# moble/scri

Hardware: AMD Instinct MI355X
Metric: timesteps/sec for full BMS transform, l_max=16, 1e5 steps; fp64 (higher is better)
Workload: dtype f64

## Files before the change

### scri_amd/csrc/engine.h

```cpp
#pragma once
#include <algorithm>
#include <array>
#include <cmath>
#include <chrono>
#include <cstdarg>
#include <cstdio>
#include <cstdlib>
#include <cstring>
#include <functional>
#include <map>
#include <new>
#include <string>
#include <thread>
#include <vector>

#include "../../include/scri_amd.h"
#include "kernels.h"
#include "pixel_math.h"
#include "wigner.h"

using namespace bms;

#define BMS_INTERNAL __attribute__((visibility("hidden")))

// ... 87 lines not shown
  int64_t n = 0, lo = 0, hi = 0, j0 = 0, j1 = 0;
  std::vector<double> host;
  const double* pending = nullptr;
  bool walked = false, regular = true;
  double* d_x = nullptr;
  BsplineTable* d_tab = nullptr;
  BsplineForward* d_fwd = nullptr;
};
struct PixelCache {
  bool valid = false, in_use = false, hit = false;
  uint64_t gen = 0;
  std::string key;
  PixelTables T;
  DevPixel D;
  bool B_valid = false;
  int B_spin = 0, B_ell_min = 0, B_ell_max = 0, B_cols = 0;
  double* d_B = nullptr;
  bool B5_valid = false, B5_sigma = false;
  int B5_ell_max = 0, B5_cols = 0;
  double* d_B5[5] = {nullptr, nullptr, nullptr, nullptr, nullptr};
  bool win_valid = false, win_abd = false;
  uint64_t win_tgen = 0, win_pgen = 0;
  int64_t win_lo = 0, win_hi = 0;
};

struct bms_ctx {
  int device = 0;
  hipStream_t own_stream = nullptr;
  hipStream_t stream = nullptr;
  hipStream_t aux = nullptr;
  std::string err;
  RouteOptions opt;
  uint64_t ws_limit = 96ull << 30;
  bool ws_limit_set = false;
  uint64_t sticky_limit = 0;
  int sticky_left = 0;
  unsigned long long* d_eval_stats = nullptr;
  uint64_t eval_tiles = 0;
  bool alloc_failed = false;
  std::map<std::string, DevBuf> bufs;
  std::vector<Slab> slabs;
  int delta_lmax = -1;
  int delta_mfma_lmax = -1;
  uint64_t rot_launches[3] = {0, 0, 0};
  int rot_valu_waves = 0;
  hipStream_t pipe_up = nullptr, pipe_down = nullptr;
// ... 5 lines not shown
  size_t pix_back_cap = 0;
  hipEvent_t ev_tables = nullptr, ev_aux_done = nullptr;
  double* rot_ring_dev = nullptr;
  int rot_ring_next = 0;
  std::map<std::pair<int, int>, RotResPlan> rot_res_plans;
  int n_cu = 0;
  std::map<std::string, std::pair<std::array<int, 6>, AnalysisPlan>> plans;
  std::map<std::array<int, 5>, SynthesisPlan> syn_plans;
  double ring_key[9] = {0, 0, 0, 0, 0, 0, 0, 0, 0};
  int ring_verdict = -1;
  std::vector<double> ring_thetas;
  std::map<std::array<int, 5>, std::pair<std::vector<double>, SynthesisPlan>> syn_plans_axis;
  bool timing = false;
  struct Timed {
    int tag;
    hipEvent_t a, b;
  };
  std::vector<Timed> timed;
  std::vector<hipEvent_t> event_pool;
  double tag_ms[BMS_TAG_COUNT] = {0};
  long long tag_calls[BMS_TAG_COUNT] = {0};
  TimeAxisCache tcache;
  PixelCache pcache;
};

static inline void note_alloc_failure(bms_ctx* c) {
  if (c) c->alloc_failed = true;
}

struct ScopedTimer {
  bms_ctx* c;
  int tag;
  hipStream_t stream;
  hipEvent_t a = nullptr, b = nullptr;
  static hipEvent_t get(bms_ctx* c) {
    if (!c->event_pool.empty()) {
      hipEvent_t e = c->event_pool.back();
      c->event_pool.pop_back();
      return e;
    }
    hipEvent_t e = nullptr;
    (void)hipEventCreate(&e);
    return e;
  }
  ScopedTimer(bms_ctx* c_, int tag_, hipStream_t stream_ = nullptr) : c(c_), tag(tag_), stream(stream_ ? stream_ : c_->stream) {
    if (c->timing) {
// ... 283 lines not shown
  c->tcache.in_use = c->tcache.hit = false;
  c->tcache.pending = nullptr;
  c->pcache.in_use = c->pcache.hit = false;
}
inline int reuse_tag(const bms_shard* sh) { return 1 + ((sh && sh->col_parts > 1 && sh->col_part >= 0) ? 1 + (sh->col_part & 0x7fff) + ((sh->col_parts & 0x7fff) << 15) : 0); }
struct KnotTables {
  double* d_x = nullptr;
  SplineTable* d_tab = nullptr;
  BsplineTable* d_bstab = nullptr;
  BsplineForward* d_bsfwd = nullptr;
  bool times_ahead = false;
  bool axis_known = false;
};
struct ChunkPlan {
  int64_t chunk = 0;
  int spline_tile = SPLINE_TILE;
};
BMS_INTERNAL int knot_tables_ahead(bms_ctx* c, const double* t, int64_t n, const bms_shard* sh, int64_t t_lo, int64_t t_hi, KnotTables& kt);
BMS_INTERNAL int knot_tables_of_call(bms_ctx* c, const double* t, int64_t n, int64_t t_lo, int64_t t_hi, int64_t row0, int64_t rows_avail, bool bsg, PieceTables* shared, KnotTables& kt);
BMS_INTERNAL int refuse_sharded_graded_axis(bms_ctx* c, bool regular_mesh, const bms_shard* sh, int64_t n);
BMS_INTERNAL int plan_chunks(bms_ctx* c, uint64_t ws_limit, double bytes_per_row, int64_t n_new, bool regular_mesh, int64_t n, const char* how_many, int n_cols, ChunkPlan& P);
BMS_INTERNAL int chunk_rows(bms_ctx* c, const PixelTables& T, const double* t, int64_t n, bool regular_mesh, int64_t c0, int64_t c1, int64_t row0, int64_t rows_avail, int64_t& g0, int64_t& g1);
BMS_INTERNAL int rotate_into_grid_frame(bms_ctx* c, const bms_transformation* tr, double* data, int64_t rows, int64_t ld, int ell_min, int ell_max);
BMS_INTERNAL int rotated_input_in_grid_frame(bms_ctx* c, const bms_transformation* tr, const char* name, int mem, const double** d_data, int64_t rows, int64_t ld, int ell_min, int ell_max);
BMS_INTERNAL int spline_eval_args(bms_ctx* c, const KnotTables& kt, const PixelTables& T, int cA, int cB, const double* t, int64_t n, int64_t g0, int64_t g1, int64_t c0, int64_t c1,
                                  double* out, long long ldo, long long ldg, SplineEval& ev);
BMS_INTERNAL void time_axis_commit(bms_ctx* c, bool walked, bool regular);
BMS_INTERNAL void drop_setup_caches(bms_ctx* c);
BMS_INTERNAL bool cached_window(bms_ctx* c, bool abd, int64_t& i_lo, int64_t& i_hi);
BMS_INTERNAL void keep_window(bms_ctx* c, bool abd, int64_t i_lo, int64_t i_hi);
BMS_INTERNAL int stage_in(bms_ctx* c, const char* name, const void* src, int mem, size_t bytes, const double** dev);
BMS_INTERNAL void time_window(int64_t n, const bms_shard* sh, int64_t& lo, int64_t& hi);
BMS_INTERNAL int validate_transformation(bms_ctx* c, int64_t n, const double* t, const bms_transformation* tr, int64_t n_min);
BMS_INTERNAL int walk_time_axis(bms_ctx* c, const double* t, int64_t lo, int64_t hi, bool* regular);
BMS_INTERNAL int validate_common(bms_ctx* c, int64_t n, const double* t, const bms_transformation* tr, int64_t lo = 0, int64_t hi = -1,
                           bool* regular = nullptr, int64_t n_min = 4);
BMS_INTERNAL int spline_tile_for(const double* x, int64_t n);
BMS_INTERNAL BsplineSpread skew_spread(const PixelTables& T, int cA, int cB, const double* x_host);
BMS_INTERNAL int eval_search_halfwidth(const PixelTables& T, int cA, int cB, const double* x_host, int64_t g0, int64_t g1);
BMS_INTERNAL bool large_synthesis_route(const bms_ctx* c, int n_theta, int n_phi, int ell_min, int ell_max);
BMS_INTERNAL bool axis_boost_pays(const bms_ctx* c, int n_modes, int n_theta, int n_phi);
BMS_INTERNAL bool separable_rotor_grid(const bms_transformation* tr, std::vector<double>& thetas, bool axis_boost_off = false);
BMS_INTERNAL bool separable_rotor_grid(bms_ctx* c, const bms_transformation* tr, std::vector<double>& thetas);
BMS_INTERNAL int build_synthesis(bms_ctx* c, int n_theta, int n_phi, int spin, int ell_min, int ell_max, SynthesisPlan& P,
                           const std::vector<double>* thetas = nullptr);
BMS_INTERNAL int run_synthesis(bms_ctx* c, const SynthesisPlan& P, const double* A, long long lda, long long rows, const double* off, double* Y,
                         long long ldy, const double* scale = nullptr);
BMS_INTERNAL int column_plan(const bms_ctx* c, const bms_transformation* tr, int n_out);
BMS_INTERNAL int device_pixel_tables(bms_ctx* c, const bms_transformation* tr, PixelTables& T, int mode, int spin, int cw,
                               const std::vector<cplx>* coef0, const std::vector<cplx>* coef1, const cplx cv[4], DevPixel& D,
                               int plan, hipStream_t PS = nullptr,
                               const std::function<int(hipStream_t, const DevPixel&, int)>& behind_tables = nullptr,
                               const std::function<void()>& while_waiting = nullptr, int reuse = 0);
BMS_INTERNAL int tables_and_window(bms_ctx* c, const bms_transformation* tr, const double* t, int64_t n, bool abd, PixelTables& T, int64_t& i_lo,
                                   int64_t& i_hi);
BMS_INTERNAL int column_range(bms_ctx* c, const bms_shard* sh, int n_cols, int& cA, int& cB);
BMS_INTERNAL int part_analysis_matrix(bms_ctx* c, const AnalysisPlan& A, const char* name, int n_cols, const int* col_of_pixel,
                                double** d_At, long long* ld_at);
BMS_INTERNAL uint64_t eval_tile_count(long long rows, int n_cols, int step);
BMS_INTERNAL int rotate_impl(bms_ctx* c, void* data, int mem, int64_t n_times, int64_t ld, int ell_min, int ell_max, const void* spinors, bool series,
                             bool sync_after = true);
```

### scri_amd/csrc/engine_modes.hip

```cpp
#include "engine.h"

constexpr int SYN_EVAL_MIN_ELL = 15;

struct PointwiseWM {
  const double* d_off = nullptr;
  const double* d_scale = nullptr;
  int n_aux = 0;
  double coeff[4];
  int power[4];
  const double *d_alpha = nullptr, *d_xa = nullptr, *d_xb = nullptr;
};

extern "C" int bms_transform_modes(bms_ctx* c, const bms_wm_input* in, const bms_transformation* tr, double* t_out,
                                   void* data_out, int64_t* n_times_out) try {
  return bms_transform_modes_shard(c, in, tr, nullptr, t_out, data_out, n_times_out, nullptr);
} BMS_CATCH(c)

extern "C" int bms_shard_plan(bms_ctx* c, const double* t, int64_t n, const bms_transformation* tr, int64_t out_i0,
                              int64_t out_i1, int64_t need_rows[2], int64_t window[2]) try {
  if (!t || !tr || !need_rows || !window) return fail(c, BMS_ERR_INVALID, "NULL argument");
  int rc = validate_common(c, n, t, tr);
  if (rc) return rc;
  PixelTables T;
  build_pixel_tables(tr, T);
// ... 349 lines not shown
    const bool want_syn_eval = c->opt.on(OPT_SYNTHESIS_EVAL) || (!c->opt.on(OPT_NO_SYNTHESIS_EVAL) && in->ell_max >= SYN_EVAL_MIN_ELL);
    if (sep && no_boost && bs && syn.nt != 0 && rows_avail >= 8 && in->t && want_syn_eval &&
        synthesis_eval_supported(syn.g, syn.nt, &se_lds, &se_nph, &se_rr, &se_xw)) {
      double bound = 0.0;
      for (int l = 1; l <= lst; ++l)
        for (int m = -l; m <= l; ++m) {
          const cplx a = st[LM_index(l, m, 0)];
          bound += std::sqrt(a.re * a.re + a.im * a.im) * std::sqrt((2 * l + 1) / (4 * M_PI));
        }
      const int64_t r0 = row0, r1 = row0 + rows_avail;
      double dx = (in->t[r1 - 1] - in->t[r0]) / (double)(r1 - 1 - r0);
      for (int64_t k = r0; k + 64 < r1; k += 64) dx = std::min(dx, (in->t[k + 64] - in->t[k]) / 64.0);
      syn_eval = dx > 0.0 && 2.0 * bound / dx <= (se_xw >= 1024 ? 384.0 : 160.0);
      for (int l = 0; l <= lst && !coef0.empty(); ++l)
        for (int m = -l; m <= l; ++m) {
          const cplx a = coef0[LM_index(l, m, 0)];
          if ((a.re != 0 || a.im != 0) && (l < in->ell_min || l > in->ell_max)) syn_eval = false;
        }
    }
  }
  std::vector<int> term_col;
  std::vector<double> term_val;
  double* d_Ac = nullptr;
  if (gemm_eval || syn_eval) {
    if ((rc = dev_buf_t(c, "Afull", (size_t)rows_avail * ld_af, &d_Ac))) return rc;
    if (c->opt.on(OPT_TWO_SWEEPS)) {
      if ((rc = dev_buf_t(c, "Afwd", (size_t)rows_avail * ld_af, &d_Af))) return rc;
      TIMED(c, BMS_TAG_SPLINE_FORWARD, launch_bspline_forward_modes(S, F[0].d_data, F[0].ld * 2, n_modes, d_Af, ld_af, row0, rows_avail, n, kt.d_bsfwd,
                                                                    SPLINE_TILE, SPLINE_HALO, 1));
      TIMED(c, BMS_TAG_SPLINE_BACKWARD, launch_bspline_backward_modes(S, d_Af, ld_af, n_modes + 1, d_Ac, ld_af, row0, rows_avail, kt.d_bstab, SPLINE_TILE, SPLINE_HALO));
    } else
      TIMED(c, BMS_TAG_SPLINE_FORWARD, launch_bspline_solve_modes(S, F[0].d_data, F[0].ld * 2, n_modes, d_Ac, ld_af, row0, rows_avail, kt.d_bsfwd, kt.d_bstab, 1));
    if (syn_eval && !coef0.empty()) {
      for (int l = in->ell_min; l <= std::min(lst, in->ell_max); ++l)
        for (int m = -l; m <= l; ++m) {
          const cplx a = coef0[LM_index(l, m, 0)];
          if (a.re == 0 && a.im == 0) continue;
          term_col.push_back(LM_index(l, m, in->ell_min));
          term_val.push_back(a.re);
          term_val.push_back(a.im);
        }
      if (!term_col.empty()) {
        void *vc, *vv;
        if ((rc = upload(c, "term_col", term_col.data(), sizeof(int) * term_col.size(), &vc))) return rc;
        if ((rc = upload(c, "term_val", term_val.data(), sizeof(double) * term_val.size(), &vv))) return rc;
        TIMED(c, BMS_TAG_POINTWISE, launch_sub_const_modes(S, d_Ac, ld_af, rows_avail, (int)term_col.size(), (const int*)vc, (const double*)vv, n_modes));
      }
    }
  } else if (bs && rows_avail > 0) {
    if ((rc = dev_buf_t(c, "Afwd", (size_t)rows_avail * ld_af, &d_Af))) return rc;
    TIMED(c, BMS_TAG_SPLINE_FORWARD, launch_bspline_forward_modes(S, F[0].d_data, F[0].ld * 2, n_modes, d_Af, ld_af, row0, rows_avail, n, kt.d_bsfwd,
                                                                  SPLINE_TILE, SPLINE_HALO, 1));
  }
  trace.mark("elimination / solve on the modes (enqueue)");
  if (sep && (rc = rotate_into_grid_frame(c, tr, syn_eval ? d_Ac : d_Af, rows_avail, ld_af / 2, in->ell_min, in->ell_max))) return rc;
  SynthesisPlan syn_f[5];
  bool sep_fields = false;
  if (!bs && rows_avail >= 1 && !(sh && sh->col_parts > 1) && tr->n_theta >= 3 && !c->opt.on(OPT_NO_SEPARABLE_SYNTHESIS) &&
      (no_boost || (axis_boost_pays(c, n_modes, tr->n_theta, tr->n_phi) && separable_rotor_grid(c, tr, ring_theta)))) {
    sep_fields = true;
    for (int fi = 0; fi < 1 + (psi ? in->n_aux : 0) && sep_fields; ++fi) {
      const int f_spin = fi ? in->aux_spin[fi - 1] : s, f_lo = fi ? in->aux_ell_min[fi - 1] : in->ell_min, f_hi = fi ? in->aux_ell_max[fi - 1] : in->ell_max;
      if (f_lo < 0 || f_hi < f_lo) {
        sep_fields = false;
        break;
      }
      if ((rc = build_synthesis(c, tr->n_theta, tr->n_phi, f_spin, f_lo, f_hi, syn_f[fi], no_boost ? nullptr : &ring_theta))) return rc;
      sep_fields = syn_f[fi].large;
    }
  }
  PixelTables T;
  DevPixel DP;
  const int col_plan = (grid_out || sep || sep_fields) ? 0 : column_plan(c, tr, n_out);
  bool B_built = false;
  if (shared && c->piece_tables_valid) {
    if (shared->col_plan != col_plan)
      return fail(c, BMS_ERR_UNSUPPORTED, "a piece of the pipelined call chose another synthesis route than the first one (column plan %d vs %d)",
                  col_plan, shared->col_plan);
// ... 252 lines not shown
```

### scri_amd/csrc/engine_rotate.hip

```cpp
#include "engine.h"


constexpr int ROT_RING = 64;

static hipError_t copy_block(char* host, int64_t ld, double* dev, int64_t n_modes, int64_t n_times, int blocks, int k, bool up, hipStream_t s) {
  const int64_t r0 = n_times * k / blocks, rows = n_times * (k + 1) / blocks - r0;
  const size_t row_bytes = (size_t)n_modes * 16, pitch = (size_t)ld * 16;
  char* h = host + (size_t)r0 * pitch;
  return up ? hipMemcpy2DAsync(dev, row_bytes, h, pitch, row_bytes, (size_t)rows, hipMemcpyHostToDevice, s)
            : hipMemcpy2DAsync(h, pitch, dev, row_bytes, row_bytes, (size_t)rows, hipMemcpyDeviceToHost, s);
}
int rotate_impl(bms_ctx* c, void* data, int mem, int64_t n_times, int64_t ld, int ell_min, int ell_max, const void* spinors, bool series,
                bool sync_after) {
  if (!c) return BMS_ERR_INVALID;
  if (!valid_mem(mem)) return fail(c, BMS_ERR_INVALID, "mem is BMS_HOST or BMS_DEVICE, got %d", mem);
  HIP_TRY(c, hipSetDevice(c->device));
  if (n_times < 0 || ell_min < 0 || ell_max < ell_min) return fail(c, BMS_ERR_INVALID, "bad sizes");
  if (ell_max > MAX_ELL) return fail(c, BMS_ERR_UNSUPPORTED, "ell_max = %d is beyond %d", ell_max, MAX_ELL);
  const int64_t n_modes = LM_total_size(ell_min, ell_max);
  if (ld < n_modes) return fail(c, BMS_ERR_INVALID, "row stride %lld smaller than %lld modes", (long long)ld, (long long)n_modes);
  if (n_times == 0) return BMS_OK;
  if (!data) return fail(c, BMS_ERR_INVALID, "NULL data");
  struct Segment {
    int lo, hi, kind;
    RotResPlan plan;
    size_t lds;
    const double* tab;
  };
  std::vector<Segment> segs;
  int rc = BMS_OK;
  {
    const bool allow_res = !c->opt.on(OPT_ROTATE_VALU) && !c->opt.on(OPT_ROTATE_STAGED) && ld * 256 <= 0x7ffe0000LL;
    int l = ell_min;
    while (l <= ell_max) {
      Segment sg{};
      bool placed = false;
// ... 12 lines not shown
        }
      }
      if (!placed) {
        sg.lo = l;
        sg.hi = ell_max;
        sg.kind = (rotate_mfma_supported(ell_max) && !c->opt.on(OPT_ROTATE_VALU)) ? 1 : 2;
        if (sg.kind == 2 && rotate_waves_per_block(ell_max) < 1)
          return fail(c, BMS_ERR_UNSUPPORTED, "ell_max=%d too large for the rotation kernels", ell_max);
      }
      segs.push_back(sg);
      l = sg.hi + 1;
    }
  }
  const double* d_delta = nullptr;
  const long long* d_off = nullptr;
  if (segs.back().kind != 0) {
    rc = segs.back().kind == 1 ? ensure_delta_mfma(c, ell_max, &d_delta, &d_off) : ensure_delta(c, ell_max, &d_delta, &d_off);
    if (rc) return rc;
  }
  double* d_data = (double*)data;
  const double* d_rot = (const double*)spinors;
  const size_t data_bytes = ((size_t)(n_times - 1) * ld + n_modes) * 16;
  const size_t rot_bytes = (series ? (size_t)n_times : 1) * 32;
  auto launch_segments = [&](double* base, int64_t rows, int64_t pitch, const double* rot) -> int {
    for (const Segment& sg : segs) {
      double* seg_data = base + 2 * ((long long)sg.lo * sg.lo - (long long)ell_min * ell_min);
      if (sg.kind == 0)
        TIMED(c, BMS_TAG_ROTATE, launch_rotate_modes_resident(c->stream, seg_data, rows, pitch, rot, series ? 4 : 0, sg.tab, sg.plan, sg.lds, nullptr, c->n_cu));
      else if (sg.kind == 1)
        TIMED(c, BMS_TAG_ROTATE, launch_rotate_modes_mfma(c->stream, seg_data, rows, pitch, sg.lo, sg.hi, rot, series ? 4 : 0, d_delta, d_off));
      else
        TIMED(c, BMS_TAG_ROTATE, launch_rotate_modes(c->stream, seg_data, rows, pitch, sg.lo, sg.hi, rot, series ? 4 : 0, d_delta, d_off, &c->rot_valu_waves));
      if (rows > 0) ++c->rot_launches[sg.kind];
    }
    return BMS_OK;
  };
  const size_t row_bytes = (size_t)n_modes * 16;
  int blocks = c->opt.on(OPT_NO_ROTATE_PIPELINE) ? 1 : (int)std::min<size_t>(16, (size_t)n_times * row_bytes / (12u << 20));
  if (const char* e = BMS_PROBE_ENV("SCRI_AMD_ROTATE_BLOCKS")) blocks = atoi(e);
  if (mem == BMS_HOST && blocks >= 2 && n_times >= 64 * blocks) {
    const int64_t rows_max = (n_times + blocks - 1) / blocks;
    double* d_buf[2];
    if ((rc = dev_buf_t(c, "rot_pipe0", (size_t)rows_max * n_modes * 2, &d_buf[0]))) return rc;
    if ((rc = dev_buf_t(c, "rot_pipe1", (size_t)rows_max * n_modes * 2, &d_buf[1]))) return rc;
    const double* d_r = nullptr;
    {
      double* r = nullptr;
      if ((rc = dev_buf_t(c, "rot_spinors", rot_bytes / 8, &r))) return rc;
      HIP_TRY(c, hipMemcpyAsync(r, spinors, rot_bytes, hipMemcpyHostToDevice, c->stream));
      d_r = r;
    }
    const char* err = "rotation of a host series in blocks";
    return run_host_pipeline(
        c, 0, blocks, true, false, err, err,
        [&](int k, int slot) { return copy_block((char*)data, ld, d_buf[slot], n_modes, n_times, blocks, k, true, c->pipe_up); },
        [&](int k, int slot) {
// ... 157 lines not shown
```

### scri_amd/csrc/engine_tables.hip

```cpp
#include "engine.h"


void build_rotor_grid(const double fr[4], const double v[3], int n_theta, int n_phi, std::vector<Quat>& R) {
  R.resize((size_t)n_theta * n_phi);
  const Quat frq = {fr[0], fr[1], fr[2], fr[3]};
  const BoostSpec bs = make_boost_spec(v);
  for (int j = 0; j < n_theta; ++j)
    for (int k = 0; k < n_phi; ++k) R[(size_t)j * n_phi + k] = pixel_rotor(frq, bs, j, k, n_theta, n_phi);
}

void theta_quadrature_weights(int n_theta, std::vector<double>& q) {
  const int M = 2 * n_theta - 2;
  q.assign(n_theta, 0.0);
  for (int j = 0; j < n_theta; ++j) {
    const double th = M_PI * j / (n_theta - 1);
    double E = 0.0;
    for (int p = -M / 2 + 1; p <= M / 2; ++p)
      if ((p & 1) == 0) E += 2.0 / (1.0 - (double)p * p) * std::cos(p * th);
    q[j] = (2 * M_PI / M) * E * ((j == 0 || j == n_theta - 1) ? 1.0 : 2.0);
  }
}

template <class T>
void delta_matrix(int ell, std::vector<double>& D ) {
// ... 453 lines not shown
    K.walked = false, K.regular = true;
    K.pending = t + lo;
    K.in_use = true;
  }
  return BMS_OK;
}

void time_axis_commit(bms_ctx* c, bool walked, bool regular) {
  TimeAxisCache& K = c->tcache;
  if (!K.in_use) return;
  if (K.pending) {
    K.host.assign(K.pending, K.pending + (K.hi - K.lo));
    K.pending = nullptr;
    K.valid = true;
  }
  if (walked && K.valid) K.walked = true, K.regular = regular;
}

void drop_setup_caches(bms_ctx* c) {
  c->tcache.valid = c->tcache.in_use = c->tcache.hit = false;
  c->tcache.pending = nullptr;
  c->pcache.valid = c->pcache.in_use = c->pcache.hit = false;
  c->pcache.B_valid = c->pcache.B5_valid = c->pcache.win_valid = false;
}

static bool window_keepable(const bms_ctx* c) {
  const TimeAxisCache& A = c->tcache;
  return A.in_use && c->pcache.in_use && A.lo == 0 && A.hi == A.n;
}
bool cached_window(bms_ctx* c, bool abd, int64_t& i_lo, int64_t& i_hi) {
  const PixelCache& P = c->pcache;
  if (!window_keepable(c) || !c->tcache.hit || !P.hit || !P.win_valid || P.win_abd != abd || P.win_tgen != c->tcache.gen || P.win_pgen != P.gen)
    return false;
  i_lo = P.win_lo, i_hi = P.win_hi;
  return true;
}
void keep_window(bms_ctx* c, bool abd, int64_t i_lo, int64_t i_hi) {
  PixelCache& P = c->pcache;
  if (!window_keepable(c)) return;
  P.win_valid = true, P.win_abd = abd, P.win_tgen = c->tcache.gen, P.win_pgen = P.gen, P.win_lo = i_lo, P.win_hi = i_hi;
}

int stage_in(bms_ctx* c, const char* name, const void* src, int mem, size_t bytes, const double** dev) {
  if (mem == BMS_DEVICE) {
    *dev = (const double*)src;
    return BMS_OK;
// ... 480 lines not shown
  return BMS_OK;
}

int chunk_rows(bms_ctx* c, const PixelTables& T, const double* t, int64_t n, bool regular_mesh, int64_t c0, int64_t c1, int64_t row0,
               int64_t rows_avail, int64_t& g0, int64_t& g1) {
  g0 = 0, g1 = n;
  if (regular_mesh) needed_rows(T, t, n, c0, c1, g0, g1);
  if (g0 < row0 || g1 > row0 + rows_avail)
    return fail(c, BMS_ERR_INVALID,
                "shard holds rows [%lld, %lld) but outputs [%lld, %lld) need rows [%lld, %lld): halo too small "
                "(use bms_shard_plan)",
                (long long)row0, (long long)(row0 + rows_avail), (long long)c0, (long long)c1, (long long)g0, (long long)g1);
  return BMS_OK;
}

static bool identity_rotor(const double* q) { return q[0] == 1.0 && q[1] == 0.0 && q[2] == 0.0 && q[3] == 0.0; }
int rotate_into_grid_frame(bms_ctx* c, const bms_transformation* tr, double* data, int64_t rows, int64_t ld, int ell_min, int ell_max) {
  const double* q = tr->frame_rotation;
  if (identity_rotor(q)) return BMS_OK;
  const double sp[4] = {q[0], q[3], q[2], q[1]};
  return rotate_impl(c, data, BMS_DEVICE, rows, ld, ell_min, ell_max, sp, false, false);
}

int rotated_input_in_grid_frame(bms_ctx* c, const bms_transformation* tr, const char* name, int mem, const double** d_data, int64_t rows, int64_t ld,
                                int ell_min, int ell_max) {
  double* d_copy = const_cast<double*>(*d_data);
  if (mem == BMS_DEVICE && !identity_rotor(tr->frame_rotation)) {
    int rc;
    if ((rc = dev_buf_t(c, name, (size_t)rows * ld * 2, &d_copy))) return rc;
    HIP_TRY(c, hipMemcpyAsync(d_copy, *d_data, (size_t)rows * ld * 16, hipMemcpyDeviceToDevice, c->stream));
    *d_data = d_copy;
  }
  return rotate_into_grid_frame(c, tr, d_copy, rows, ld, ell_min, ell_max);
}

int spline_eval_args(bms_ctx* c, const KnotTables& kt, const PixelTables& T, int cA, int cB, const double* t, int64_t n, int64_t g0, int64_t g1,
                     int64_t c0, int64_t c1, double* out, long long ldo, long long ldg, SplineEval& ev) {
  ev.table = kt.d_bstab, ev.x = kt.d_x, ev.tt = T.tt, ev.g0 = g0, ev.n_knots = n;
  ev.i_lo = c0, ev.i_hi = c1, ev.out = out, ev.ldo = ldo;
  ev.search_halfwidth = eval_search_halfwidth(T, cA, cB, t, g0, g1);
  ev.inv_dx = (g1 - g0 >= 2 && t[g1 - 1] > t[g0]) ? (double)(g1 - 1 - g0) / (t[g1 - 1] - t[g0]) : 0.0;
  ev.side = nullptr, ev.side_ld = ldg;
  if (!c->d_eval_stats) {
    HIP_TRY(c, hipMalloc(&c->d_eval_stats, 16));
    HIP_TRY(c, hipMemsetAsync(c->d_eval_stats, 0, 16, c->stream));
  }
// ... 7 lines not shown
```

### scri_amd/csrc/kernels.h

```cpp
#pragma once
#include <algorithm>
#include <vector>
#include <hip/hip_runtime.h>
#include <stdint.h>

#include "env.h"

#include <map>
#include <mutex>
#include <utility>

namespace bms {

constexpr long long GRID_Y_MAX = 65535;

inline int lds_per_workgroup(int dev) {
  int lds = 0, v = 0;
  if (hipDeviceGetAttribute(&v, hipDeviceAttributeSharedMemPerBlockOptin, dev) == hipSuccess) lds = std::max(lds, v);
  if (hipDeviceGetAttribute(&v, hipDeviceAttributeMaxSharedMemoryPerBlock, dev) == hipSuccess) lds = std::max(lds, v);
  (void)hipGetLastError();
  if (lds <= 64 * 1024) lds = 160 * 1024;
  return lds;
}

// ... 162 lines not shown
                                       long long g0, long long n_rows, long long n_knots, const double* x,
                                       const SplineTable* table, int tile, int halo, const double* base,
                                       const double* skew_a, const double* skew_b, double tt, long long i_lo,
                                       long long i_hi, double* out, long long ldo);

struct BsplineTable {
  double m[16];
  double G, D;
  double x;
  double pad;
};
struct BsplineForward {
  double P, A, E, x;
};
hipError_t launch_bspline_table(hipStream_t stream, const double* x, long long n, BsplineTable* table, BsplineForward* fwd,
                                long long j_lo , long long j0, long long j1);
hipError_t launch_bspline_forward_modes(hipStream_t stream, const double* A, long long lda, int n_modes, double* Aout,
                                        long long ldo, long long g0, long long n_rows, long long n_knots,
                                        const BsplineForward* table, int tile, int halo, int with_ones);
hipError_t launch_bspline_backward_modes(hipStream_t stream, const double* A, long long lda, int n_cols, double* Aout, long long ldo,
                                         long long g0, long long n_rows, const BsplineTable* table, int tile, int halo);
hipError_t launch_bspline_solve_modes(hipStream_t stream, const double* A, long long lda, int n_modes, double* Aout, long long ldo,
                                      long long g0, long long n_rows, const BsplineForward* fwd, const BsplineTable* table, int with_ones);
struct AbdGrids;
hipError_t launch_abd_mix_forward(hipStream_t stream, const AbdGrids& Y, const AbdGrids& R, long long ld, int n_cols, long long g0,
                                  long long n_rows, const BsplineForward* table, int tile, int halo, const double* alpha,
                                  const double* ethk_over_k, const double* eth_alpha, const double* etheth_alpha,
                                  const double* inv_k, const double* inv_k3, int n_fields = 6 );
hipError_t launch_negated_row(hipStream_t stream, const double* off, double* row, int n);
struct BsplineSpread {
  double skew_rate_range, skew_offset_range;
  const double* x;
};
hipError_t launch_bspline_backward_eval(hipStream_t stream, const double* C, long long ld, int n_cols, long long g0,
                                        long long n_rows, long long n_knots, const double* x, const BsplineTable* table,
                                        int tile, int halo, const double* base, const double* skew_a, const double* skew_b,
                                        double tt, long long i_lo, long long i_hi, double* out, long long ldo, const BsplineSpread* spread = nullptr);

hipError_t launch_spline_slopes(hipStream_t stream, const double* R, double* S, long long ld, int n_cols, long long n,
                                const SplineTable* table, int tile, int halo);
long long spline_prefix_carry_size(long long n, int n_cols);
hipError_t launch_spline_prefix_levels(hipStream_t stream, const double* Y, const double* S, long long ld, int n_cols, long long n,
                                       const double* x, double* Pall, long long level_stride, double* carry, int levels);
hipError_t launch_spline_antiderivative_eval(hipStream_t stream, const double* Y, const double* S, const double* Pall, long long level_stride,
                                             long long ld, int n_cols, long long n, const double* x, const double* x_new, long long n_new,
                                             int k, double* out, long long ldo);
// ... 132 lines not shown
```

### scri_amd/csrc/kernels_bspline.hip

```cpp
#include <cstdlib>
#include "wigner.h"
#include <algorithm>
#include <cmath>

#include "kernels.h"

namespace bms {

__device__ __forceinline__ void bspline_local(const double* __restrict__ x, long long n, long long j, double P[16]) {
  long long f = j - 1;
  if (f < 0) f = 0;
  if (f > n - 4) f = n - 4;
  const long long mu = f + 3;
  const double xj = x[j];
  auto tau = [&](long long k) { return k <= 3 ? x[0] : (k >= n ? x[n - 1] : x[k - 2]); };
  double prev[4][4], cur[4][4];
#pragma unroll
  for (int i = 0; i < 4; ++i)
#pragma unroll
    for (int d = 0; d < 4; ++d) prev[i][d] = 0.0;
  prev[0][0] = 1.0;
#pragma unroll
  for (int d = 1; d <= 3; ++d) {
#pragma unroll
// ... 200 lines not shown
#pragma unroll
    for (int g = 0; g < 4; ++g) {
      r[g] = ld2(j - g);
      gd[g] = ldt(j - g);
    }
#pragma unroll
    for (int g = 0; g < 4; ++g) step(j - g, r[g], gd[g]);
  }
  for (; j >= jA; --j) step(j, ld2(j), ldt(j));
}

hipError_t launch_bspline_backward_modes(hipStream_t stream, const double* A, long long lda, int n_cols, double* Aout, long long ldo,
                                         long long g0, long long n_rows, const BsplineTable* table, int tile, int halo) {
  if (n_rows <= 0 || n_cols <= 0) return hipSuccess;
  static const int tile_env = BMS_PROBE_ENV("SCRI_AMD_BSPLINE_TILE_FWD") ? atoi(BMS_PROBE_ENV("SCRI_AMD_BSPLINE_TILE_FWD")) : 0;
  tile = tile_env > 0 ? tile_env : tile;
  const long long n_tiles = (n_rows + tile - 1) / tile;
  if (n_tiles > GRID_Y_MAX) return hipErrorInvalidValue;
  dim3 grid((n_cols + 63) / 64, (unsigned)n_tiles);
  hipLaunchKernelGGL(bspline_backward_modes_kernel, grid, dim3(64), 0, stream, A, lda, n_cols, Aout, ldo, g0, n_rows, table, tile, halo);
  return hipGetLastError();
}

template <int TT, int HH>
__global__ __launch_bounds__(64) __attribute__((amdgpu_waves_per_eu(2, 2))) void bspline_solve_modes_kernel(
    const double* __restrict__ A, long long lda, int n_modes, double* __restrict__ O, long long ldo, long long g0, long long n_rows,
    const BsplineForward* __restrict__ fwd, const BsplineTable* __restrict__ table, int with_ones) {
  constexpr int NR = TT + 2 * HH;
  __shared__ __attribute__((aligned(16))) double fw[NR][4];
  __shared__ __attribute__((aligned(16))) double bw[NR][2];
  const int lane = threadIdx.x;
  const int n_real = 2 * (n_modes + with_ones), ncb = (n_real + 63) / 64;
  const long long n_tiles = (n_rows + TT - 1) / TT, per_xcd = (n_tiles + 7) / 8;
  const long long q = blockIdx.x >> 3;
  const long long tile = (long long)(blockIdx.x & 7) * per_xcd + q / ncb;
  if (q / ncb >= per_xcd || tile >= n_tiles) return;
  const int p = (int)(q % ncb) * 64 + lane;
  const long long jA = g0 + tile * TT, jend = g0 + n_rows;
  const long long j0 = jA - HH;
  for (int r = lane; r < NR; r += 64) {
    const long long j = j0 + r;
    const bool ok = j >= g0 && j < jend;
    double2 pa = {1.0, 0.0}, ex = {0.0, 0.0}, gd = {0.0, 0.0};
    if (ok) {
      pa = *reinterpret_cast<const double2*>(&fwd[j].P);
      ex = *reinterpret_cast<const double2*>(&fwd[j].E);
      gd = *reinterpret_cast<const double2*>(&table[j].G);
    }
    *reinterpret_cast<double2*>(&fw[r][0]) = pa;
    fw[r][2] = ex.x;
    *reinterpret_cast<double2*>(&bw[r][0]) = gd;
  }
  const bool live = p < n_real;
  const bool ones = with_ones && p >= 2 * n_modes;
  const double one_value = (p & 1) ? 0.0 : 1.0;
  const double* ap = A + (live && !ones ? p : 0);
  double v[NR];
#pragma unroll
  for (int r = 0; r < NR; ++r) {
    const long long j = j0 + r;
    const bool ok = j >= g0 && j < jend;
    v[r] = ok ? (ones ? one_value : ap[(j - g0) * lda]) : 0.0;
  }
  __syncthreads();
#pragma unroll
  for (int r = 0; r < NR; ++r) {
    const double2 pa = *reinterpret_cast<const double2*>(&fw[r][0]);
    const double e = fw[r][2];
    const double c1 = r >= 1 ? v[r - 1] : 0.0, c2 = r >= 2 ? v[r - 2] : 0.0;
    v[r] = pa.x * v[r] - pa.y * c1 - e * c2;
  }
#pragma unroll
  for (int r = NR - 1; r >= HH; --r) {
    const double2 gd = *reinterpret_cast<const double2*>(&bw[r][0]);
    const double w0 = r + 1 < NR ? v[r + 1] : 0.0, w1 = r + 2 < NR ? v[r + 2] : 0.0;
    v[r] = v[r] - gd.x * w0 - gd.y * w1;
  }
  if (!live) return;
  double* op = O + p;
#pragma unroll
  for (int r = HH; r < HH + TT; ++r) {
    const long long j = j0 + r;
    if (j < jend) op[(j - g0) * ldo] = v[r];
  }
}

hipError_t launch_bspline_solve_modes(hipStream_t stream, const double* A, long long lda, int n_modes, double* Aout, long long ldo,
                                      long long g0, long long n_rows, const BsplineForward* fwd, const BsplineTable* table, int with_ones) {
  if (n_rows <= 0 || n_modes <= 0) return hipSuccess;
  constexpr int TT = 48, HH = 32;
  const long long ncb = (2 * (n_modes + with_ones) + 63) / 64, n_tiles = (n_rows + TT - 1) / TT, per_xcd = (n_tiles + 7) / 8;
  dim3 grid((unsigned)(8 * per_xcd * ncb));
  hipLaunchKernelGGL((bspline_solve_modes_kernel<TT, HH>), grid, dim3(64), 0, stream, A, lda, n_modes, Aout, ldo, g0, n_rows, fwd, table, with_ones);
  return hipGetLastError();
}

template <int NF>
__global__ __launch_bounds__(64) void abd_mix_forward_kernel(AbdGrids Yg, AbdGrids Rg, long long ld, int n_cols, long long g0,
                                                             long long n_rows, const BsplineForward* __restrict__ table, int tile,
                                                             int halo, const double* __restrict__ alpha,
                                                             const double* __restrict__ ethk_over_k,
                                                             const double* __restrict__ eth_alpha,
                                                             const double* __restrict__ etheth_alpha,
                                                             const double* __restrict__ inv_k, const double* __restrict__ inv_k3) {
  const int p = blockIdx.x * blockDim.x + threadIdx.x;
  if (p >= n_cols) return;
  const long long jA = g0 + (long long)blockIdx.y * tile;
// ... 387 lines not shown
```

Measured before the change: 21.78 million.

## Fuse frame rotation into B-spline solve using per-ell MFMA Wigner blocks

Adds a kernel that runs the B-spline banded solve on the mode columns and then applies the frame rotation in registers. The rotation is done as per-ell block matrix products with fp64 MFMA, so the separate rotate_into_grid_frame pass over the solved data is skipped. Rotation blocks are built once by rotating unit rows and are cached per rotor, ell range and coef0, and the constant-term subtraction uses the rotated coef0. The cost is a larger, more register-heavy solve kernel (192 threads, waves_per_eu pinned) and extra setup work when the rotation changes.

```diff
diff --git a/scri_amd/csrc/engine.h b/scri_amd/csrc/engine.h
--- a/scri_amd/csrc/engine.h
+++ b/scri_amd/csrc/engine.h
@@ -133,6 +133,18 @@
   bool win_valid = false, win_abd = false;
   uint64_t win_tgen = 0, win_pgen = 0;
   int64_t win_lo = 0, win_hi = 0;
+};
+
+struct SolveRotCache {
+  bool valid = false;
+  double q[4] = {0, 0, 0, 0};
+  int ell_min = 0, ell_max = 0;
+  std::vector<cplx> coef0;
+  std::vector<double> rows;
+  SolveRotPlan plan;
+  std::vector<int> tables;
+  SolveRot dev{};
+  const double* d_coef0_rot = nullptr;
 };
 
 struct bms_ctx {
@@ -184,6 +196,7 @@
   long long tag_calls[BMS_TAG_COUNT] = {0};
   TimeAxisCache tcache;
   PixelCache pcache;
+  SolveRotCache rcache;
 };
 
 static inline void note_alloc_failure(bms_ctx* c) {
@@ -513,6 +526,7 @@
 BMS_INTERNAL int plan_chunks(bms_ctx* c, uint64_t ws_limit, double bytes_per_row, int64_t n_new, bool regular_mesh, int64_t n, const char* how_many, int n_cols, ChunkPlan& P);
 BMS_INTERNAL int chunk_rows(bms_ctx* c, const PixelTables& T, const double* t, int64_t n, bool regular_mesh, int64_t c0, int64_t c1, int64_t row0, int64_t rows_avail, int64_t& g0, int64_t& g1);
 BMS_INTERNAL int rotate_into_grid_frame(bms_ctx* c, const bms_transformation* tr, double* data, int64_t rows, int64_t ld, int ell_min, int ell_max);
+BMS_INTERNAL int solve_rot_blocks(bms_ctx* c, const bms_transformation* tr, int ell_min, int ell_max, const std::vector<cplx>& coef0, const SolveRotCache** rot);
 BMS_INTERNAL int rotated_input_in_grid_frame(bms_ctx* c, const bms_transformation* tr, const char* name, int mem, const double** d_data, int64_t rows, int64_t ld, int ell_min, int ell_max);
 BMS_INTERNAL int spline_eval_args(bms_ctx* c, const KnotTables& kt, const PixelTables& T, int cA, int cB, const double* t, int64_t n, int64_t g0, int64_t g1, int64_t c0, int64_t c1,
                                   double* out, long long ldo, long long ldg, SplineEval& ev);
@@ -550,4 +564,4 @@
                                 double** d_At, long long* ld_at);
 BMS_INTERNAL uint64_t eval_tile_count(long long rows, int n_cols, int step);
 BMS_INTERNAL int rotate_impl(bms_ctx* c, void* data, int mem, int64_t n_times, int64_t ld, int ell_min, int ell_max, const void* spinors, bool series,
-                             bool sync_after = true);
+                             bool sync_after = true, bool set_up = false);
diff --git a/scri_amd/csrc/engine_modes.hip b/scri_amd/csrc/engine_modes.hip
--- a/scri_amd/csrc/engine_modes.hip
+++ b/scri_amd/csrc/engine_modes.hip
@@ -395,6 +395,7 @@
   std::vector<int> term_col;
   std::vector<double> term_val;
   double* d_Ac = nullptr;
+  const SolveRotCache* solve_rot = nullptr;
   if (gemm_eval || syn_eval) {
     if ((rc = dev_buf_t(c, "Afull", (size_t)rows_avail * ld_af, &d_Ac))) return rc;
     if (c->opt.on(OPT_TWO_SWEEPS)) {
@@ -402,9 +403,34 @@
       TIMED(c, BMS_TAG_SPLINE_FORWARD, launch_bspline_forward_modes(S, F[0].d_data, F[0].ld * 2, n_modes, d_Af, ld_af, row0, rows_avail, n, kt.d_bsfwd,
                                                                     SPLINE_TILE, SPLINE_HALO, 1));
       TIMED(c, BMS_TAG_SPLINE_BACKWARD, launch_bspline_backward_modes(S, d_Af, ld_af, n_modes + 1, d_Ac, ld_af, row0, rows_avail, kt.d_bstab, SPLINE_TILE, SPLINE_HALO));
-    } else
-      TIMED(c, BMS_TAG_SPLINE_FORWARD, launch_bspline_solve_modes(S, F[0].d_data, F[0].ld * 2, n_modes, d_Ac, ld_af, row0, rows_avail, kt.d_bsfwd, kt.d_bstab, 1));
-    if (syn_eval && !coef0.empty()) {
+    } else {
+      if (syn_eval && !sh && c->opt.on(OPT_SYNTHESIS_EVAL) && (rc = solve_rot_blocks(c, tr, in->ell_min, in->ell_max, coef0, &solve_rot))) return rc;
+      if (solve_rot) {
+        ScopedTimer rotation_in_the_solve(c, BMS_TAG_ROTATE);
+      }
+      if (solve_rot)
+        TIMED(c, BMS_TAG_SPLINE_FORWARD,launch_bspline_solve_rotate_modes(S, F[0].d_data, F[0].ld * 2, n_modes, d_Ac, ld_af, row0, rows_avail, kt.d_bsfwd,
+                                                                           kt.d_bstab, solve_rot->dev));
+      else
+        TIMED(c, BMS_TAG_SPLINE_FORWARD, launch_bspline_solve_modes(S, F[0].d_data, F[0].ld * 2, n_modes, d_Ac, ld_af, row0, rows_avail, kt.d_bsfwd, kt.d_bstab, 1));
+    }
+    if (syn_eval && !coef0.empty() && solve_rot) {
+      int l_lo = -1, l_hi = -1;
+      for (int l = in->ell_min; l <= std::min(lst, in->ell_max); ++l)
+        for (int m = -l; m <= l; ++m) {
+          const cplx a = coef0[LM_index(l, m, 0)];
+          if (a.re == 0 && a.im == 0) continue;
+          if (l_lo < 0) l_lo = l;
+          l_hi = l;
+        }
+      if (l_lo >= 0) {
+        for (int k = LM_index(l_lo, -l_lo, in->ell_min); k <= LM_index(l_hi, l_hi, in->ell_min); ++k) term_col.push_back(k);
+        void* vc;
+        if ((rc = upload(c, "term_col", term_col.data(), sizeof(int) * term_col.size(), &vc))) return rc;
+        TIMED(c, BMS_TAG_POINTWISE, launch_sub_const_modes(S, d_Ac, ld_af, rows_avail, (int)term_col.size(), (const int*)vc,
+                                                           solve_rot->d_coef0_rot + 2 * term_col[0], n_modes));
+      }
+    } else if (syn_eval && !coef0.empty()) {
       for (int l = in->ell_min; l <= std::min(lst, in->ell_max); ++l)
         for (int m = -l; m <= l; ++m) {
           const cplx a = coef0[LM_index(l, m, 0)];
@@ -426,7 +452,7 @@
                                                                   SPLINE_TILE, SPLINE_HALO, 1));
   }
   trace.mark("elimination / solve on the modes (enqueue)");
-  if (sep && (rc = rotate_into_grid_frame(c, tr, syn_eval ? d_Ac : d_Af, rows_avail, ld_af / 2, in->ell_min, in->ell_max))) return rc;
+  if (sep && !solve_rot && (rc = rotate_into_grid_frame(c, tr, syn_eval ? d_Ac : d_Af, rows_avail, ld_af / 2, in->ell_min, in->ell_max))) return rc;
   SynthesisPlan syn_f[5];
   bool sep_fields = false;
   if (!bs && rows_avail >= 1 && !(sh && sh->col_parts > 1) && tr->n_theta >= 3 && !c->opt.on(OPT_NO_SEPARABLE_SYNTHESIS) &&
diff --git a/scri_amd/csrc/engine_rotate.hip b/scri_amd/csrc/engine_rotate.hip
--- a/scri_amd/csrc/engine_rotate.hip
+++ b/scri_amd/csrc/engine_rotate.hip
@@ -11,7 +11,7 @@
             : hipMemcpy2DAsync(h, pitch, dev, row_bytes, row_bytes, (size_t)rows, hipMemcpyDeviceToHost, s);
 }
 int rotate_impl(bms_ctx* c, void* data, int mem, int64_t n_times, int64_t ld, int ell_min, int ell_max, const void* spinors, bool series,
-                bool sync_after) {
+                bool sync_after, bool set_up) {
   if (!c) return BMS_ERR_INVALID;
   if (!valid_mem(mem)) return fail(c, BMS_ERR_INVALID, "mem is BMS_HOST or BMS_DEVICE, got %d", mem);
   HIP_TRY(c, hipSetDevice(c->device));
@@ -70,16 +70,17 @@
   const double* d_rot = (const double*)spinors;
   const size_t data_bytes = ((size_t)(n_times - 1) * ld + n_modes) * 16;
   const size_t rot_bytes = (series ? (size_t)n_times : 1) * 32;
+  const int tag = set_up ? BMS_TAG_SETUP : BMS_TAG_ROTATE;
   auto launch_segments = [&](double* base, int64_t rows, int64_t pitch, const double* rot) -> int {
     for (const Segment& sg : segs) {
       double* seg_data = base + 2 * ((long long)sg.lo * sg.lo - (long long)ell_min * ell_min);
       if (sg.kind == 0)
-        TIMED(c, BMS_TAG_ROTATE, launch_rotate_modes_resident(c->stream, seg_data, rows, pitch, rot, series ? 4 : 0, sg.tab, sg.plan, sg.lds, nullptr, c->n_cu));
+        TIMED(c, tag, launch_rotate_modes_resident(c->stream, seg_data, rows, pitch, rot, series ? 4 : 0, sg.tab, sg.plan, sg.lds, nullptr, c->n_cu));
       else if (sg.kind == 1)
-        TIMED(c, BMS_TAG_ROTATE, launch_rotate_modes_mfma(c->stream, seg_data, rows, pitch, sg.lo, sg.hi, rot, series ? 4 : 0, d_delta, d_off));
+        TIMED(c, tag, launch_rotate_modes_mfma(c->stream, seg_data, rows, pitch, sg.lo, sg.hi, rot, series ? 4 : 0, d_delta, d_off));
       else
-        TIMED(c, BMS_TAG_ROTATE, launch_rotate_modes(c->stream, seg_data, rows, pitch, sg.lo, sg.hi, rot, series ? 4 : 0, d_delta, d_off, &c->rot_valu_waves));
-      if (rows > 0) ++c->rot_launches[sg.kind];
+        TIMED(c, tag, launch_rotate_modes(c->stream, seg_data, rows, pitch, sg.lo, sg.hi, rot, series ? 4 : 0, d_delta, d_off, &c->rot_valu_waves));
+      if (rows > 0 && !set_up) ++c->rot_launches[sg.kind];
     }
     return BMS_OK;
   };
diff --git a/scri_amd/csrc/engine_tables.hip b/scri_amd/csrc/engine_tables.hip
--- a/scri_amd/csrc/engine_tables.hip
+++ b/scri_amd/csrc/engine_tables.hip
@@ -499,6 +499,7 @@
   c->tcache.pending = nullptr;
   c->pcache.valid = c->pcache.in_use = c->pcache.hit = false;
   c->pcache.B_valid = c->pcache.B5_valid = c->pcache.win_valid = false;
+  c->rcache.valid = false;
 }
 
 static bool window_keepable(const bms_ctx* c) {
@@ -1025,6 +1026,62 @@
   return rotate_impl(c, data, BMS_DEVICE, rows, ld, ell_min, ell_max, sp, false, false);
 }
 
+int solve_rot_blocks(bms_ctx* c, const bms_transformation* tr, int ell_min, int ell_max, const std::vector<cplx>& coef0, const SolveRotCache** rot) {
+  *rot = nullptr;
+  const double* q = tr->frame_rotation;
+  if (identity_rotor(q)) return BMS_OK;
+  SolveRotCache& K = c->rcache;
+  const bool keep = !c->opt.on(OPT_NO_PLAN_CACHE);
+  if (keep && K.valid && std::memcmp(K.q, q, sizeof K.q) == 0 && K.ell_min == ell_min && K.ell_max == ell_max && K.coef0.size() == coef0.size() &&
+      (coef0.empty() || std::memcmp(K.coef0.data(), coef0.data(), sizeof(cplx) * coef0.size()) == 0)) {
+    *rot = &K;
+    return BMS_OK;
+  }
+  SolveRotPlan plan;
+  if (!solve_rot_plan(ell_min, ell_max, plan)) return BMS_OK;
+  if (!K.rows.empty()) HIP_TRY(c, hipStreamSynchronize(c->stream));
+  K.valid = false;
+  K.plan = plan;
+  const int n_modes = LM_total_size(ell_min, ell_max), n_unit = 2 * ell_max + 1;
+  K.rows.assign((size_t)(n_unit + 1) * n_modes * 2, 0.0);
+  for (int r = 0; r < n_unit; ++r) {
+    const int mp = r - ell_max;
+    for (int l = std::max(ell_min, std::abs(mp)); l <= ell_max; ++l) K.rows[((size_t)r * n_modes + LM_index(l, mp, ell_min)) * 2] = 1.0;
+  }
+  for (int l = ell_min; l <= ell_max && (size_t)(l + 1) * (l + 1) <= coef0.size(); ++l)
+    for (int m = -l; m <= l; ++m) {
+      const cplx a = coef0[LM_index(l, m, 0)];
+      K.rows[((size_t)n_unit * n_modes + LM_index(l, m, ell_min)) * 2] = a.re;
+      K.rows[((size_t)n_unit * n_modes + LM_index(l, m, ell_min)) * 2 + 1] = a.im;
+    }
+  const int ng = plan.n_groups();
+  K.tables.clear();
+  K.tables.insert(K.tables.end(), plan.group_col.begin(), plan.group_col.end());
+  K.tables.insert(K.tables.end(), plan.group_job.begin(), plan.group_job.end());
+  static_assert(sizeof(SolveRotJob) == 8 * sizeof(int), "jobs travel as ints");
+  const size_t job0 = (K.tables.size() + 7) / 8 * 8;
+  K.tables.resize(job0 + 8 * plan.jobs.size());
+  std::memcpy(K.tables.data() + job0, plan.jobs.data(), sizeof(SolveRotJob) * plan.jobs.size());
+  void *v_rows, *v_tab;
+  double* d_D;
+  int rc;
+  if ((rc = upload(c, "rc_rows", K.rows.data(), sizeof(double) * K.rows.size(), &v_rows))) return rc;
+  if ((rc = upload(c, "rc_tables", K.tables.data(), sizeof(int) * K.tables.size(), &v_tab))) return rc;
+  if ((rc = dev_buf_t(c, "rc_D", (size_t)plan.block_off.back(), &d_D))) return rc;
+  const double sp[4] = {q[0], q[3], q[2], q[1]};
+  if ((rc = rotate_impl(c, v_rows, BMS_DEVICE, n_unit + 1, n_modes, ell_min, ell_max, sp, false, false, true))) return rc;
+  TIMED(c, BMS_TAG_SETUP, launch_solve_rot_blocks(c->stream, (const double*)v_rows, n_modes, ell_min, ell_max, d_D));
+  const int* d_tab = (const int*)v_tab;
+  K.dev.group_col = d_tab, K.dev.group_job = d_tab + ng + 1, K.dev.jobs = reinterpret_cast<const SolveRotJob*>(d_tab + job0);
+  K.dev.D = d_D, K.dev.n_groups = ng;
+  K.d_coef0_rot = (const double*)v_rows + (size_t)n_unit * n_modes * 2;
+  std::memcpy(K.q, q, sizeof K.q);
+  K.ell_min = ell_min, K.ell_max = ell_max, K.coef0 = coef0;
+  K.valid = keep;
+  *rot = &K;
+  return BMS_OK;
+}
+
 int rotated_input_in_grid_frame(bms_ctx* c, const bms_transformation* tr, const char* name, int mem, const double** d_data, int64_t rows, int64_t ld,
                                 int ell_min, int ell_max) {
   double* d_copy = const_cast<double*>(*d_data);
diff --git a/scri_amd/csrc/kernels.h b/scri_amd/csrc/kernels.h
--- a/scri_amd/csrc/kernels.h
+++ b/scri_amd/csrc/kernels.h
@@ -208,6 +208,71 @@
                                          long long g0, long long n_rows, const BsplineTable* table, int tile, int halo);
 hipError_t launch_bspline_solve_modes(hipStream_t stream, const double* A, long long lda, int n_modes, double* Aout, long long ldo,
                                       long long g0, long long n_rows, const BsplineForward* fwd, const BsplineTable* table, int with_ones);
+constexpr int SOLVE_ROT_WAVES = 3, SOLVE_ROT_COLS = 64 * SOLVE_ROT_WAVES;
+constexpr int SOLVE_ROT_KSTEPS = 17;
+inline int solve_rot_kpad(int l) { return (4 * l + 2 + 3) & ~3; }
+inline int solve_rot_npad(int l) { return (4 * l + 2 + 15) & ~15; }
+struct SolveRotJob {
+  int a_col;
+  int k_real, kpad;
+  int n0, n_valid;
+  int d_off, d_pitch;
+  int pad;
+};
+struct SolveRotPlan {
+  std::vector<int> group_col;
+  std::vector<int> group_job;
+  std::vector<SolveRotJob> jobs;
+  std::vector<long long> block_off;
+  int n_groups() const { return (int)group_col.size() - 1; }
+};
+inline bool solve_rot_plan(int ell_min, int ell_max, SolveRotPlan& P) {
+  P = SolveRotPlan{};
+  if (ell_min < 0 || ell_max < ell_min || 4 * ell_max + 2 + 2 > SOLVE_ROT_COLS || solve_rot_kpad(ell_max) > 4 * SOLVE_ROT_KSTEPS) return false;
+  P.block_off.assign(ell_max - ell_min + 2, 0);
+  for (int l = ell_min; l <= ell_max; ++l) P.block_off[l - ell_min + 1] = P.block_off[l - ell_min] + (long long)solve_rot_kpad(l) * solve_rot_npad(l);
+  if (P.block_off.back() > 0x7fffffffLL) return false;
+  std::vector<int> first_l;
+  int room = SOLVE_ROT_COLS - 2;
+  for (int l = ell_max; l >= ell_min; --l) {
+    const int w = 4 * l + 2;
+    if (l == ell_max || w > room) {
+      if (l != ell_max) room = SOLVE_ROT_COLS;
+      first_l.push_back(l);
+    } else
+      first_l.back() = l;
+    room -= w;
+  }
+  const int n_real = 2 * ((ell_max + 1) * (ell_max + 1) - ell_min * ell_min + 1);
+  P.group_col.push_back(0);
+  P.group_job.push_back(0);
+  for (int g = (int)first_l.size() - 1; g >= 0; --g) {
+    const int lo = first_l[g], hi = g ? first_l[g - 1] - 1 : ell_max;
+    const int col0 = 2 * (lo * lo - ell_min * ell_min);
+    for (int l = lo; l <= hi; ++l)
+      for (int n0 = 0; n0 < 4 * l + 2; n0 += 16) {
+        SolveRotJob j{};
+        j.a_col = 2 * (l * l - ell_min * ell_min) - col0;
+        j.k_real = 4 * l + 2, j.kpad = solve_rot_kpad(l);
+        j.n0 = j.a_col + n0, j.n_valid = std::min(16, 4 * l + 2 - n0);
+        j.d_off = (int)P.block_off[l - ell_min] + n0, j.d_pitch = solve_rot_npad(l);
+        P.jobs.push_back(j);
+      }
+    P.group_col.push_back(g ? 2 * (first_l[g - 1] * first_l[g - 1] - ell_min * ell_min) : n_real);
+    P.group_job.push_back((int)P.jobs.size());
+  }
+  return true;
+}
+struct SolveRot {
+  const int* group_col;
+  const int* group_job;
+  const SolveRotJob* jobs;
+  const double* D;
+  int n_groups;
+};
+hipError_t launch_solve_rot_blocks(hipStream_t stream, const double* rows, int n_modes, int ell_min, int ell_max, double* D);
+hipError_t launch_bspline_solve_rotate_modes(hipStream_t stream, const double* A, long long lda, int n_modes, double* Aout, long long ldo,
+                                             long long g0, long long n_rows, const BsplineForward* fwd, const BsplineTable* table, const SolveRot& rot);
 struct AbdGrids;
 hipError_t launch_abd_mix_forward(hipStream_t stream, const AbdGrids& Y, const AbdGrids& R, long long ld, int n_cols, long long g0,
                                   long long n_rows, const BsplineForward* table, int tile, int halo, const double* alpha,
diff --git a/scri_amd/csrc/kernels_bspline.hip b/scri_amd/csrc/kernels_bspline.hip
--- a/scri_amd/csrc/kernels_bspline.hip
+++ b/scri_amd/csrc/kernels_bspline.hip
@@ -246,6 +246,40 @@
   return hipGetLastError();
 }
 
+template <int NR>
+__device__ __forceinline__ void solve_stage_factors(double (*fw)[4], double (*bw)[2], int tid, int n_threads, long long j0, long long g0, long long jend,
+                                                    const BsplineForward* __restrict__ fwd, const BsplineTable* __restrict__ table) {
+  for (int r = tid; r < NR; r += n_threads) {
+    const long long j = j0 + r;
+    const bool ok = j >= g0 && j < jend;
+    double2 pa = {1.0, 0.0}, ex = {0.0, 0.0}, gd = {0.0, 0.0};
+    if (ok) {
+      pa = *reinterpret_cast<const double2*>(&fwd[j].P);
+      ex = *reinterpret_cast<const double2*>(&fwd[j].E);
+      gd = *reinterpret_cast<const double2*>(&table[j].G);
+    }
+    *reinterpret_cast<double2*>(&fw[r][0]) = pa;
+    fw[r][2] = ex.x;
+    *reinterpret_cast<double2*>(&bw[r][0]) = gd;
+  }
+}
+template <int NR, int HH>
+__device__ __forceinline__ void solve_sweeps(double (&v)[NR], const double (*fw)[4], const double (*bw)[2]) {
+#pragma unroll
+  for (int r = 0; r < NR; ++r) {
+    const double2 pa = *reinterpret_cast<const double2*>(&fw[r][0]);
+    const double e = fw[r][2];
+    const double c1 = r >= 1 ? v[r - 1] : 0.0, c2 = r >= 2 ? v[r - 2] : 0.0;
+    v[r] = pa.x * v[r] - pa.y * c1 - e * c2;
+  }
+#pragma unroll
+  for (int r = NR - 1; r >= HH; --r) {
+    const double2 gd = *reinterpret_cast<const double2*>(&bw[r][0]);
+    const double w0 = r + 1 < NR ? v[r + 1] : 0.0, w1 = r + 2 < NR ? v[r + 2] : 0.0;
+    v[r] = v[r] - gd.x * w0 - gd.y * w1;
+  }
+}
+
 template <int TT, int HH>
 __global__ __launch_bounds__(64) __attribute__((amdgpu_waves_per_eu(2, 2))) void bspline_solve_modes_kernel(
     const double* __restrict__ A, long long lda, int n_modes, double* __restrict__ O, long long ldo, long long g0, long long n_rows,
@@ -262,19 +296,7 @@
   const int p = (int)(q % ncb) * 64 + lane;
   const long long jA = g0 + tile * TT, jend = g0 + n_rows;
   const long long j0 = jA - HH;
-  for (int r = lane; r < NR; r += 64) {
-    const long long j = j0 + r;
-    const bool ok = j >= g0 && j < jend;
-    double2 pa = {1.0, 0.0}, ex = {0.0, 0.0}, gd = {0.0, 0.0};
-    if (ok) {
-      pa = *reinterpret_cast<const double2*>(&fwd[j].P);
-      ex = *reinterpret_cast<const double2*>(&fwd[j].E);
-      gd = *reinterpret_cast<const double2*>(&table[j].G);
-    }
-    *reinterpret_cast<double2*>(&fw[r][0]) = pa;
-    fw[r][2] = ex.x;
-    *reinterpret_cast<double2*>(&bw[r][0]) = gd;
-  }
+  solve_stage_factors<NR>(fw, bw, lane, 64, j0, g0, jend, fwd, table);
   const bool live = p < n_real;
   const bool ones = with_ones && p >= 2 * n_modes;
   const double one_value = (p & 1) ? 0.0 : 1.0;
@@ -287,19 +309,7 @@
     v[r] = ok ? (ones ? one_value : ap[(j - g0) * lda]) : 0.0;
   }
   __syncthreads();
-#pragma unroll
-  for (int r = 0; r < NR; ++r) {
-    const double2 pa = *reinterpret_cast<const double2*>(&fw[r][0]);
-    const double e = fw[r][2];
-    const double c1 = r >= 1 ? v[r - 1] : 0.0, c2 = r >= 2 ? v[r - 2] : 0.0;
-    v[r] = pa.x * v[r] - pa.y * c1 - e * c2;
-  }
-#pragma unroll
-  for (int r = NR - 1; r >= HH; --r) {
-    const double2 gd = *reinterpret_cast<const double2*>(&bw[r][0]);
-    const double w0 = r + 1 < NR ? v[r + 1] : 0.0, w1 = r + 2 < NR ? v[r + 2] : 0.0;
-    v[r] = v[r] - gd.x * w0 - gd.y * w1;
-  }
+  solve_sweeps<NR, HH>(v, fw, bw);
   if (!live) return;
   double* op = O + p;
 #pragma unroll
@@ -307,6 +317,143 @@
     const long long j = j0 + r;
     if (j < jend) op[(j - g0) * ldo] = v[r];
   }
+}
+
+template <int TT, int HH, int RC, int NJ>
+__global__ __launch_bounds__(SOLVE_ROT_COLS) __attribute__((amdgpu_waves_per_eu(2, 2))) void bspline_solve_rotate_modes_kernel(
+    const double* __restrict__ A, long long lda, int n_modes, double* __restrict__ O, long long ldo, long long g0, long long n_rows,
+    const BsplineForward* __restrict__ fwd, const BsplineTable* __restrict__ table, const int* __restrict__ group_col,
+    const int* __restrict__ group_job, const SolveRotJob* __restrict__ jobs, const double* __restrict__ Dm, int n_groups) {
+  constexpr int NR = TT + 2 * HH, LDS_PITCH = SOLVE_ROT_COLS + 2, KS = SOLVE_ROT_KSTEPS;
+  static_assert(TT % RC == 0 && RC % 16 == 0, "whole accumulator tiles");
+  __shared__ __attribute__((aligned(16))) double fw[NR][4];
+  __shared__ __attribute__((aligned(16))) double bw[NR][2];
+  __shared__ __attribute__((aligned(16))) double S[RC][LDS_PITCH];
+  const int tid = threadIdx.x;
+  const int ncb = n_groups;
+  const long long n_tiles = (n_rows + TT - 1) / TT, per_xcd = (n_tiles + 7) / 8;
+  const long long q = blockIdx.x >> 3;
+  const long long tile = (long long)(blockIdx.x & 7) * per_xcd + q / ncb;
+  if (q / ncb >= per_xcd || tile >= n_tiles) return;
+  const int grp = (int)(q % ncb);
+  const int col0 = group_col[grp], n_cols = group_col[grp + 1] - col0;
+  const long long jA = g0 + tile * TT, jend = g0 + n_rows;
+  const long long j0 = jA - HH;
+  solve_stage_factors<NR>(fw, bw, tid, SOLVE_ROT_COLS, j0, g0, jend, fwd, table);
+  const int p = col0 + tid;
+  const bool live = tid < n_cols;
+  const bool ones = p >= 2 * n_modes;
+  const double one_value = (p & 1) ? 0.0 : 1.0;
+  const double* ap = A + (live && !ones ? p : 0);
+  double v[NR];
+#pragma unroll
+  for (int r = 0; r < NR; ++r) {
+    const long long j = j0 + r;
+    const bool ok = j >= g0 && j < jend;
+    v[r] = ok ? (ones ? one_value : ap[(j - g0) * lda]) : 0.0;
+  }
+  __syncthreads();
+  solve_sweeps<NR, HH>(v, fw, bw);
+  if (live && ones) {
+#pragma unroll
+    for (int r = 0; r < TT; ++r)
+      if (jA + r < jend) O[(jA + r - g0) * ldo + p] = v[HH + r];
+  }
+  const int wave = __builtin_amdgcn_readfirstlane(tid >> 6), lane = tid & 63;
+  const int fi = lane & 15, fk = lane >> 4;
+  const int job_end = group_job[grp + 1];
+  typedef double v4d __attribute__((ext_vector_type(4)));
+#pragma unroll
+  for (int c0 = 0; c0 < TT; c0 += RC) {
+    if (c0) __syncthreads();
+#pragma unroll
+    for (int r = 0; r < RC; ++r) S[r][tid] = live ? v[HH + c0 + r] : 0.0;
+    for (int jb0 = group_job[grp] + wave, batch = 0; batch == 0 || jb0 < job_end; jb0 += NJ * SOLVE_ROT_WAVES, ++batch) {
+      double b[NJ][KS];
+#pragma unroll
+      for (int i = 0; i < NJ; ++i) {
+        const int jb = jb0 + i * SOLVE_ROT_WAVES;
+        const SolveRotJob J = jobs[__builtin_amdgcn_readfirstlane(jb < job_end ? jb : job_end - 1)];
+        const int kpad = jb < job_end ? J.kpad : 0;
+        const double* bp = Dm + J.d_off + fk * J.d_pitch + fi;
+#pragma unroll
+        for (int s = 0; s < KS; ++s) b[i][s] = 4 * s < kpad ? bp[s * 4 * J.d_pitch] : 0.0;
+      }
+      if (batch == 0) __syncthreads();
+#pragma unroll
+      for (int i = 0; i < NJ; ++i) {
+        const int jb = jb0 + i * SOLVE_ROT_WAVES;
+        if (jb >= job_end) break;
+        const SolveRotJob J = jobs[__builtin_amdgcn_readfirstlane(jb)];
+        v4d acc[RC / 16];
+#pragma unroll
+        for (int c = 0; c < RC / 16; ++c) acc[c] = v4d{0.0, 0.0, 0.0, 0.0};
+        const double* sp = &S[fi][J.a_col + fk];
+        const int k_last = J.k_real - fk;
+#pragma unroll
+        for (int s = 0; s < KS; ++s) {
+          if (4 * s >= J.kpad) break;
+#pragma unroll
+          for (int c = 0; c < RC / 16; ++c) {
+            double a = sp[16 * c * LDS_PITCH + 4 * s];
+            a = 4 * s < k_last ? a : 0.0;
+            acc[c] = __builtin_amdgcn_mfma_f64_16x16x4f64(a, b[i][s], acc[c], 0, 0, 0);
+          }
+        }
+        if (fi < J.n_valid) {
+          double* op = O + col0 + J.n0 + fi;
+#pragma unroll
+          for (int c = 0; c < RC / 16; ++c)
+#pragma unroll
+            for (int r = 0; r < 4; ++r) {
+              const long long j = jA + c0 + 16 * c + fk + 4 * r;
+              if (j < jend) op[(j - g0) * ldo] = acc[c][r];
+            }
+        }
+      }
+    }
+  }
+}
+
+__global__ __launch_bounds__(256) void solve_rot_blocks_kernel(const double* __restrict__ rows, int n_modes, int ell_min, int ell_max, double* __restrict__ D,
+                                                               int total) {
+  const int e = blockIdx.x * blockDim.x + threadIdx.x;
+  if (e >= total) return;
+  int l = ell_min, off = 0;
+  for (;; ++l) {
+    const int sz = ((4 * l + 2 + 3) & ~3) * ((4 * l + 2 + 15) & ~15);
+    if (e < off + sz) break;
+    off += sz;
+  }
+  const int npad = (4 * l + 2 + 15) & ~15, k = (e - off) / npad, n = (e - off) % npad;
+  double val = 0.0;
+  if (k < 4 * l + 2 && n < 4 * l + 2) {
+    const int mp = (k >> 1) - l, m = (n >> 1) - l;
+    const double* d = rows + 2 * ((long long)(mp + ell_max) * n_modes + (l * l - ell_min * ell_min) + (m + l));
+    val = (k & 1) == (n & 1) ? d[0] : ((k & 1) ? -d[1] : d[1]);
+  }
+  D[e] = val;
+}
+
+hipError_t launch_solve_rot_blocks(hipStream_t stream, const double* rows, int n_modes, int ell_min, int ell_max, double* D) {
+  long long total = 0;
+  for (int l = ell_min; l <= ell_max; ++l) total += (long long)solve_rot_kpad(l) * solve_rot_npad(l);
+  if (total <= 0 || total > 0x7fffffffLL) return hipErrorInvalidValue;
+  hipLaunchKernelGGL(solve_rot_blocks_kernel, dim3((unsigned)((total + 255) / 256)), dim3(256), 0, stream, rows, n_modes, ell_min, ell_max, D, (int)total);
+  return hipGetLastError();
+}
+
+hipError_t launch_bspline_solve_rotate_modes(hipStream_t stream, const double* A, long long lda, int n_modes, double* Aout, long long ldo,
+                                             long long g0, long long n_rows, const BsplineForward* fwd, const BsplineTable* table, const SolveRot& rot) {
+  if (n_rows <= 0 || n_modes <= 0) return hipSuccess;
+  if (rot.n_groups <= 0) return hipErrorInvalidValue;
+  constexpr int TT = 48, HH = 32;
+  const long long n_tiles = (n_rows + TT - 1) / TT, per_xcd = (n_tiles + 7) / 8;
+  if (8 * per_xcd * rot.n_groups > 0x7fffffffLL) return hipErrorInvalidValue;
+  dim3 grid((unsigned)(8 * per_xcd * rot.n_groups));
+  hipLaunchKernelGGL((bspline_solve_rotate_modes_kernel<TT, HH, 48, 5>), grid, dim3(SOLVE_ROT_COLS), 0, stream, A, lda, n_modes, Aout, ldo, g0, n_rows, fwd, table,
+                     rot.group_col, rot.group_job, rot.jobs, rot.D, rot.n_groups);
+  return hipGetLastError();
 }
 
 hipError_t launch_bspline_solve_modes(hipStream_t stream, const double* A, long long lda, int n_modes, double* Aout, long long ldo,
```

Measured after the change: 21.78 million, median of 2. Within noise of the previous version (+0.0%).
